# BraveGroup/DCD

Measured on NVIDIA B200. Metric: objects/sec (edge solve + GMW aggregate), higher is better.
Workload: dtype f32

## Files before the change

### dcd_b200/csrc/gmw_mlp_fused.cu

```cuda
#include <type_traits>
#include "gmw_tc_common.cuh"

#ifndef DCD_FUSED_STAT_SLEEP
#define DCD_FUSED_STAT_SLEEP 40
#endif
#ifndef DCD_FUSED_CONV_FINAL
#define DCD_FUSED_CONV_FINAL 1
#endif
#ifndef DCD_FUSED_POLL_GRACE
#define DCD_FUSED_POLL_GRACE 500
#endif
#ifndef DCD_FUSED_DONE_SLEEP
#define DCD_FUSED_DONE_SLEEP 20
#endif

namespace dcd {
#ifdef DCD_FUSED_TRACE
__device__ long long g_trace[12288];
__device__ int g_trace_n[3];
#ifndef DCD_FUSED_TRACE_CTA
#define DCD_FUSED_TRACE_CTA 0
#endif
#ifndef DCD_FUSED_TRACE_WARP
#define DCD_FUSED_TRACE_WARP 0
#endif
#define TR_DECL const bool trace_on = blockIdx.x == DCD_FUSED_TRACE_CTA && (warp == DCD_FUSED_TRACE_WARP || warp == FCONV_WARPS || warp == FCONV_WARPS + 1); int tr_k = 0;
#define TR(slot, tag)                                                       \
    do {                                                                    \
        if (trace_on && lane == 0 && tr_k < 2048) {                         \
            g_trace[(slot) * 4096 + 2 * tr_k] = (tag);                      \
            g_trace[(slot) * 4096 + 2 * tr_k + 1] = clock64();              \
            ++tr_k;                                                         \
            g_trace_n[slot] = tr_k;                                         \
        }                                                                   \
    } while (0)
#else
#define TR_DECL
#define TR(slot, tag) do { } while (0)
#endif
#if defined(DCD_FUSED_TRACE) && DCD_FUSED_TRACE + 0 >= 2
#define TRF(slot, tag) TR(slot, tag)
#else
#define TRF(slot, tag) do { } while (0)
#endif
namespace {

constexpr int FCS = 24;
constexpr int FOBJ = 3;
constexpr int FCONV_WARPS = 12;
constexpr int FCONV_THREADS = 32 * FCONV_WARPS;
constexpr int FTHREADS = FCONV_THREADS + 128;
constexpr int FSUB = 48;
constexpr int FES_MAX = 112;
constexpr uint32_t FT_W = 384;
constexpr uint32_t FB_SBO = 128;
constexpr uint32_t FB_LBO = 768;
constexpr uint32_t FB_PART = 16 * FB_LBO;

constexpr size_t SMF_X = 0;
constexpr size_t SMF_B = SMF_X + (size_t)FOBJ * FES_MAX * CH * sizeof(float);
constexpr size_t SMF_PART = SMF_B + 4 * FB_PART;
constexpr size_t SMF_BAR = SMF_PART + (FOBJ * 3 * CH + 64) * sizeof(float2);
constexpr size_t kFusedSmem = SMF_BAR + 128;
static_assert(kFusedSmem <= 232448, "shared memory budget");
static_assert(FOBJ * 6 * FES_MAX * sizeof(float) <= 4 * FB_PART, "edge features are staged in the operand buffers");
static_assert(FOBJ * FES_MAX <= FCONV_THREADS, "one converter thread per staged edge");
enum { BAR_FULL0 = 0, BAR_FULL1 = 1, BAR_DONE0 = 2, BAR_DONE1 = 3, BAR_PDONE = 4, BAR_WREADY = 5, BAR_STAT0 = 6, BAR_COUNT = 9 };
enum { NB_PART0 = 5, NB_STATW = 8 };
constexpr int FSTAT_THREADS = 96;
constexpr int NB_THREADS = FCONV_THREADS + FSTAT_THREADS;

__device__ __forceinline__ void st_flagged(float2* dst, float a, float b, uint32_t flag) {
    const uint32_t bits = (__float_as_uint(b) & 0x7fffffffu) | (flag << 31);
    const unsigned long long w = ((unsigned long long)bits << 32) | (unsigned long long)__float_as_uint(a);
    asm volatile("st.relaxed.gpu.global.b64 [%0], %1;" ::"l"(dst), "l"(w) : "memory");
}
__device__ __forceinline__ float2 ld_volatile_f2(const float2* p) {
    float2 v;
    unsigned long long w;
    asm volatile("ld.relaxed.gpu.global.b64 %0, [%1];" : "=l"(w) : "l"(p) : "memory");
    v.x = __uint_as_float((uint32_t)w);
    v.y = __uint_as_float((uint32_t)(w >> 32));
    return v;
}
__device__ __forceinline__ void ld_weights8(const uint32_t* p, uint32_t* r) {
    asm volatile("ld.global.nc.L2::evict_last.v8.b32 {%0, %1, %2, %3, %4, %5, %6, %7}, [%8];"
                 : "=r"(r[0]), "=r"(r[1]), "=r"(r[2]), "=r"(r[3]), "=r"(r[4]), "=r"(r[5]), "=r"(r[6]), "=r"(r[7])
                 : "l"(p));
}
__device__ __forceinline__ void mbar_arrive(uint64_t* bar) {
    asm volatile("mbarrier.arrive.shared::cta.b64 _, [%0];" ::"r"(smem_u32(bar)) : "memory");
}
__device__ __forceinline__ void mbar_wait_backoff(uint64_t* bar, uint32_t parity, uint32_t ns) {
    uint32_t done;
    for (;;) {
        asm volatile("{\n\t.reg .pred p;\n\tmbarrier.try_wait.parity.shared::cta.b64 p, [%1], %2;\n\tselp.u32 %0, 1, 0, p;\n\t}"
                     : "=r"(done) : "r"(smem_u32(bar)), "r"(parity) : "memory");
        if (done) break;
        if (ns) __nanosleep(ns);
    }
}
__device__ __forceinline__ void nbar_sync(int id, int count) { asm volatile("bar.sync %0, %1;" ::"r"(id), "r"(count) : "memory"); }
__device__ __forceinline__ void nbar_arrive(int id, int count) { asm volatile("bar.arrive %0, %1;" ::"r"(id), "r"(count) : "memory"); }
__device__ __forceinline__ void conv_sync() { asm volatile("bar.sync 1, %0;" ::"n"(FCONV_THREADS) : "memory"); }

__device__ __forceinline__ void tmem_ld16(uint32_t taddr, float (&v)[16]) {
    uint32_t r[16];
    asm volatile(
        "tcgen05.ld.sync.aligned.32x32b.x16.b32 "
        "{%0, %1, %2, %3, %4, %5, %6, %7, %8, %9, %10, %11, %12, %13, %14, %15}, [%16];\n\t"
        "tcgen05.wait::ld.sync.aligned;"
        : "=r"(r[0]), "=r"(r[1]), "=r"(r[2]), "=r"(r[3]), "=r"(r[4]), "=r"(r[5]), "=r"(r[6]), "=r"(r[7]), "=r"(r[8]),
          "=r"(r[9]), "=r"(r[10]), "=r"(r[11]), "=r"(r[12]), "=r"(r[13]), "=r"(r[14]), "=r"(r[15])
        : "r"(taddr)
        : "memory");
#pragma unroll
    for (int i = 0; i < 16; ++i) v[i] = __uint_as_float(r[i]);
}

__device__ __forceinline__ void tmem_ld16_issue(uint32_t taddr, uint32_t (&r)[16]) {
    asm volatile(
        "tcgen05.ld.sync.aligned.32x32b.x16.b32 "
        "{%0, %1, %2, %3, %4, %5, %6, %7, %8, %9, %10, %11, %12, %13, %14, %15}, [%16];"
        : "=r"(r[0]), "=r"(r[1]), "=r"(r[2]), "=r"(r[3]), "=r"(r[4]), "=r"(r[5]), "=r"(r[6]), "=r"(r[7]), "=r"(r[8]),
          "=r"(r[9]), "=r"(r[10]), "=r"(r[11]), "=r"(r[12]), "=r"(r[13]), "=r"(r[14]), "=r"(r[15])
        : "r"(taddr)
        : "memory");
}
__device__ __forceinline__ void tmem_ld16_wait(uint32_t (&r)[16]) {
    asm volatile("tcgen05.wait::ld.sync.aligned;"
                 : "+r"(r[0]), "+r"(r[1]), "+r"(r[2]), "+r"(r[3]), "+r"(r[4]), "+r"(r[5]), "+r"(r[6]), "+r"(r[7]), "+r"(r[8]),
                   "+r"(r[9]), "+r"(r[10]), "+r"(r[11]), "+r"(r[12]), "+r"(r[13]), "+r"(r[14]), "+r"(r[15])
                 :
                 : "memory");
}

__device__ __forceinline__ void ffma2_bc(float& d0, float& d1, float a0, float a1, float b, float c) {
    asm("{\n\t.reg .b64 a, b, c, d;\n\tmov.b64 a, {%2, %3};\n\tmov.b64 b, {%4, %4};\n\tmov.b64 c, {%5, %5};\n\t"
        "fma.rn.f32x2 d, a, b, c;\n\tmov.b64 {%0, %1}, d;\n\t}"
        : "=f"(d0), "=f"(d1) : "f"(a0), "f"(a1), "f"(b), "f"(c));
}
__device__ __forceinline__ void fsq2_acc(float& s0, float& s1, float d0, float d1) {
    asm("{\n\t.reg .b64 d, s;\n\tmov.b64 d, {%2, %3};\n\tmov.b64 s, {%0, %1};\n\t"
        "fma.rn.f32x2 s, d, d, s;\n\tmov.b64 {%0, %1}, s;\n\t}"
        : "+f"(s0), "+f"(s1) : "f"(d0), "f"(d1));
}
__device__ __forceinline__ void fadd2_acc(float& s0, float& s1, float d0, float d1) {
    asm("{\n\t.reg .b64 d, s;\n\tmov.b64 d, {%2, %3};\n\tmov.b64 s, {%0, %1};\n\t"
        "add.rn.f32x2 s, s, d;\n\tmov.b64 {%0, %1}, s;\n\t}"
        : "+f"(s0), "+f"(s1) : "f"(d0), "f"(d1));
}

__device__ __forceinline__ uint64_t smem_desc_ns(uint32_t addr, uint32_t lbo, uint32_t sbo) {
    return (uint64_t)((addr & 0x3ffffu) >> 4) | ((uint64_t)(lbo >> 4) << 16) | ((uint64_t)(sbo >> 4) << 32) | (1ull << 46);
}

__device__ __forceinline__ void split2_neg(float v0, float v1, uint32_t& hp, uint32_t& lp) {
    asm("{\n\t.reg .f16 h0, h1;\n\t.reg .f32 l0, l1;\n\t"
        "cvt.rn.f16x2.f32 %0, %3, %2;\n\t"
        "mov.b32 {h0, h1}, %0;\n\t"
        "sub.rn.f32.f16 l0, h0, %2;\n\t"
        "sub.rn.f32.f16 l1, h1, %3;\n\t"
        "cvt.rn.f16x2.f32 %1, l1, l0;\n\t}"
        : "=&r"(hp), "=r"(lp)
        : "f"(v0), "f"(v1));
}

__device__ __forceinline__ void store_unit(unsigned char* b_hi, unsigned char* b_lo, int ch, int u, const float (&v)[16]) {
    uint32_t hp[8], lp[8];
#pragma unroll
    for (int q = 0; q < 8; ++q) split2_neg(v[2 * q], v[2 * q + 1], hp[q], lp[q]);
    const uint32_t off = (uint32_t)(2 * u) * FB_SBO + (uint32_t)(ch >> 3) * FB_LBO + (uint32_t)(ch & 7) * 16u;
    *reinterpret_cast<uint4*>(b_hi + off) = make_uint4(hp[0], hp[1], hp[2], hp[3]);
    *reinterpret_cast<uint4*>(b_hi + off + FB_SBO) = make_uint4(hp[4], hp[5], hp[6], hp[7]);
    *reinterpret_cast<uint4*>(b_lo + off) = make_uint4(lp[0], lp[1], lp[2], lp[3]);
    *reinterpret_cast<uint4*>(b_lo + off + FB_SBO) = make_uint4(lp[4], lp[5], lp[6], lp[7]);
}

__device__ __forceinline__ void issue_sub_gemm(uint32_t tmem_d, uint32_t a_hi, uint32_t a_lo, uint32_t b_hi, uint32_t b_lo, int N) {
    const uint32_t idesc = (1u << 4) | (1u << 16) | ((uint32_t)(N >> 3) << 17) | ((uint32_t)(CH >> 4) << 24);
    const uint64_t d_hi = smem_desc_ns(b_hi, FB_LBO, FB_SBO), d_lo = smem_desc_ns(b_lo, FB_LBO, FB_SBO);
    uint32_t acc = 0;
#pragma unroll
    for (int term = 0; term < 3; ++term) {
        const uint32_t a = (term == 1) ? a_lo : a_hi;
        const uint64_t d = (term == 0) ? d_lo : d_hi;
        const uint32_t id = (term == 0) ? (idesc | (1u << 14)) : idesc;
#pragma unroll
        for (int ks = 0; ks < CH / 16; ++ks) {
            umma_f16_ts(tmem_d, a + ks * 8, d + (uint64_t)((ks * 2 * FB_LBO) >> 4), id, acc);
            acc = 1;
        }
    }
}

}

__global__ void __launch_bounds__(1024) fused_prep_kernel(const float* __restrict__ p4, const float* __restrict__ p6, int depth,
                                                         const float* __restrict__ fold, float2* __restrict__ scales2,
                                                         float* __restrict__ bias2, uint32_t* __restrict__ img) {
    extern __shared__ float wf_s[];
    __shared__ float red[32];
    __shared__ float scale_s;
    const int m = blockIdx.x;
    const int j = m & 1, blk = (m >> 1) % depth, net = m / (2 * depth);
    const int cin = net == 0 ? 4 : 6;
    const float* prm = net == 0 ? p4 : p6;
    const int tid = threadIdx.x;
    if (j == 0) {
        const float* F = fold + ((int64_t)net * depth + blk) * FOLD_STRIDE;
        for (int i = tid; i < CH * CH; i += 1024) wf_s[i] = F[i];
        if (tid < CH) bias2[m * CH + tid] = F[CH * CH + tid];
    } else {
        const float* W2 = prm + blob_w(cin, blk, 2);
        for (int i = tid; i < CH * CH; i += 1024) wf_s[i] = W2[i];
        if (tid < CH) bias2[m * CH + tid] = prm[blob_b(cin, blk, 2) + tid];
    }
    __syncthreads();
    float mx = 0.f;
    for (int i = tid; i < CH * CH; i += 1024) mx = fmaxf(mx, fabsf(wf_s[i]));
    mx = warp_max(mx);
    if ((tid & 31) == 0) red[tid >> 5] = mx;
    __syncthreads();
    if (tid == 0) {
        mx = 0.f;
        for (int w = 0; w < 32; ++w) mx = fmaxf(mx, red[w]);
        int e = 0;
        if (mx > 0.f) frexpf(mx, &e);
        scales2[m] = make_float2(ldexpf(1.f, 10 - e), ldexpf(1.f, e - 10));
        scale_s = ldexpf(1.f, 10 - e);
    }
    __syncthreads();
    const float scale = scale_s;
    uint32_t* out = img + (size_t)m * CH * CH;
    for (int idx = tid; idx < CH * 64; idx += 1024) {
        const int row = idx & 127, c = idx >> 7;
        const float w0 = wf_s[(2 * c) * CH + row] * scale, w1 = wf_s[(2 * c + 1) * CH + row] * scale;
        const __half h0 = __float2half_rn(w0), h1 = __float2half_rn(w1);
        const __half l0 = __float2half_rn(w0 - __half2float(h0)), l1 = __float2half_rn(w1 - __half2float(h1));
        out[(((c >> 3)) * CH + row) * 8 + (c & 7)] = (uint32_t)__half_as_ushort(h0) | ((uint32_t)__half_as_ushort(h1) << 16);
        out[((8 + (c >> 3)) * CH + row) * 8 + (c & 7)] = (uint32_t)__half_as_ushort(l0) | ((uint32_t)__half_as_ushort(l1) << 16);
    }
}

namespace {

__global__ void __launch_bounds__(FTHREADS, 1)
mlp_fused_kernel(MlpArgs a, const float2* __restrict__ scales, const float* __restrict__ bias2, const uint32_t* __restrict__ wimg,
                 float2* xg, float* __restrict__ reg_w, float4* park) {
    const WsLayout& L = a.L;
    const int tid = threadIdx.x, lane = tid & 31;
    const int warp = __shfl_sync(0xffffffffu, tid >> 5, 0);
    const int quarter = warp & 3;
    TR_DECL
    const int ch = 32 * quarter + lane;
    const uint32_t rank = blockIdx.x % FCS, group = blockIdx.x / FCS;
    const int E = L.E, EP = L.EP, depth = L.depth;
    const int upo = (E + 16 * FCS - 1) / (16 * FCS);
    const int ES = 16 * upo;
    const int ntile = upo;
    const int nphase = 2 * depth;
#if DCD_FUSED_CONV_FINAL
    const bool conv_final = upo != 4;
#endif

    extern __shared__ __align__(1024) unsigned char smem[];
    float4* Xs = reinterpret_cast<float4*>(smem + SMF_X);
    unsigned char* Bbuf = smem + SMF_B;
    float2* pbuf = reinterpret_cast<float2*>(smem + SMF_PART);
    float2* tab_s = pbuf + FOBJ * 3 * CH;
    uint64_t* bar = reinterpret_cast<uint64_t*>(smem + SMF_BAR);
    uint32_t* tmem_ptr = reinterpret_cast<uint32_t*>(smem + SMF_BAR + 8 * BAR_COUNT);

    if (tid == 0) {
        mbar_init(bar + BAR_FULL0, FCONV_WARPS);
        mbar_init(bar + BAR_FULL1, FCONV_WARPS);
        mbar_init(bar + BAR_DONE0, 1);
        mbar_init(bar + BAR_DONE1, 1);
        mbar_init(bar + BAR_PDONE, 1);
        mbar_init(bar + BAR_WREADY, 4);
        for (int o = 0; o < FOBJ; ++o) mbar_init(bar + BAR_STAT0 + o, 3);
        asm volatile("fence.mbarrier_init.release.cluster;" ::: "memory");
    }
    if (tid < 9) {
        const int o = tid / 3, k = tid % 3;
        const int vld = max(0, min(ES, E - (int)rank * ES));
        int nq = 0;
        for (int u = o * upo; u < (o + 1) * upo; ++u)
            if ((u - o * upo) % 3 == k) nq += max(0, min(16, vld - 16 * (u - o * upo)));
        tab_s[tid] = make_float2((float)nq, vld > 0 ? (float)nq / (float)vld : 0.f);
        tab_s[9 + tid] = make_float2(nq > 0 ? 1.0f / (float)nq : 0.f, 0.f);
    } else if (tid >= 32 && tid < 32 + FCS) {
        const int r = tid - 32, sb = r / 8;
        const int nr = max(0, min(ES, E - r * ES));
        const int ns = max(0, min(E, (sb + 1) * 8 * ES) - min(E, sb * 8 * ES));
        tab_s[tid] = make_float2((float)nr, ns > 0 ? (float)nr / (float)ns : 0.f);
    } else if (tid >= 56 && tid < 59) {
        const int sb = tid - 56;
        const int ns = max(0, min(E, (sb + 1) * 8 * ES) - min(E, sb * 8 * ES));
        tab_s[tid] = make_float2((float)ns, (float)ns / (float)E);
    }
    if (warp == 0) tmem_alloc(tmem_ptr, 512);
    tc_fence_before();
    __syncthreads();
    tc_fence_after();
    const uint32_t tmem_base = __shfl_sync(0xffffffffu, *tmem_ptr, 0);
    const uint32_t t_lane = tmem_base + ((uint32_t)(32 * quarter) << 16);
    const int64_t ngroups = gridDim.x / FCS;
    const bool paired = reg_w != nullptr;
    const int64_t ntrip = (L.N + FOBJ - 1) / FOBJ;
    const int64_t nlist = paired ? ntrip : 2 * ntrip;
    const int64_t nmine = nlist > (int64_t)group ? (nlist - 1 - group) / ngroups + 1 : 0;
    const int64_t nd = paired ? 2 * nmine : nmine;
    auto round_trip = [&](int64_t d) { return paired ? (int64_t)group + (d >> 1) * ngroups : ((int64_t)group + d * ngroups) >> 1; };
    auto round_net = [&](int64_t d) { return paired ? (int)(d & 1) : (int)(((int64_t)group + d * ngroups) & 1); };

    if (warp >= FCONV_WARPS) {
        uint32_t wr[64];
        auto w_load = [&](int mat, int half) {
            const uint32_t* src = wimg + (size_t)mat * CH * CH + ((size_t)(half * 8) * CH + ch) * 8;
#pragma unroll
            for (int i = 0; i < 8; ++i) ld_weights8(src + (size_t)i * CH * 8, wr + 8 * i);
        };
        auto w_store = [&](int half) {
            uint32_t t[32];
#pragma unroll
            for (int i = 0; i < 32; ++i) t[i] = wr[i];
            tmem_st32(t_lane + FT_W + 64 * half, t);
#pragma unroll
            for (int i = 0; i < 32; ++i) t[i] = wr[32 + i];
            tmem_st32(t_lane + FT_W + 64 * half + 32, t);
        };
        auto w_publish = [&]() {
            tc_wait_st();
            tc_fence_before();
            __syncwarp();
            if (lane == 0) mbar_arrive(bar + BAR_WREADY);
        };
        uint32_t g = 0;
        uint32_t fpar = 0, wpar = 0, ppar = 0;
        const int nrep = warp == FCONV_WARPS + 1 ? 2 : 1;
        const float inv_em1 = 1.0f / (float)(E - 1);
        uint32_t sxc = 0;
        auto ev_row = [&](int o) {
            const uint32_t xc = (sxc >> (2 * o)) & 3u;
            return xg + ((size_t)((group * FOBJ + o) * 2 + (xc & 1u)) * FCS) * CH;
        };
        auto ev_flag = [&](int o) { return (sxc >> (2 * o + 1)) & 1u; };
        auto ev_publish = [&](int o) {
            TR(2, 700 + o);
            nbar_sync(NB_PART0 + o, NB_THREADS);
            TR(2, 710 + o);
            float2* xrow0 = ev_row(o);
            const uint32_t flag = ev_flag(o);
            float2 tb[3];
#pragma unroll
            for (int k = 0; k < 3; ++k) tb[k] = tab_s[o * 3 + k];
            const int c0 = 32 * (warp - FCONV_WARPS - 1) + lane, c1 = 96 + lane;
            float2 q[2][3];
#pragma unroll
            for (int k = 0; k < 3; ++k) {
                q[0][k] = pbuf[(o * 3 + k) * CH + c0];
                q[1][k] = pbuf[(o * 3 + k) * CH + c1];
            }
#pragma unroll
            for (int rep = 0; rep < 2; ++rep) {
                float m = 0.f, M2 = 0.f;
#pragma unroll
                for (int k = 0; k < 3; ++k) m = fmaf(tb[k].y, q[rep][k].x, m);
#pragma unroll
                for (int k = 0; k < 3; ++k) {
                    const float dd = q[rep][k].x - m;
                    if (tb[k].x > 0.f) M2 += fmaf(tb[k].x * dd, dd, q[rep][k].y);
                }
                if (rep < nrep) st_flagged(xrow0 + rank * CH + (rep ? c1 : c0), m, M2, flag);
            }
            nbar_sync(NB_STATW, FSTAT_THREADS);
            TR(2, 720 + o);
        };
        auto ev_finish = [&](int o, bool fresh) {
            const int sb = warp - FCONV_WARPS - 1;
            const float2* xrow0 = ev_row(o) + (size_t)(8 * sb) * CH + lane;
            const uint32_t flag = ev_flag(o);
            if (fresh) __nanosleep(DCD_FUSED_POLL_GRACE);
            float2 v[4][8];
            for (;;) {
#pragma unroll
                for (int q = 0; q < 4; ++q)
#pragma unroll
                    for (int r = 0; r < 8; ++r) v[q][r] = ld_volatile_f2(xrow0 + r * CH + 32 * q);
                uint32_t bad = 0;
#pragma unroll
                for (int q = 0; q < 4; ++q)
#pragma unroll
                    for (int r = 0; r < 8; ++r) bad |= (__float_as_uint(v[q][r].y) >> 31) ^ flag;
                if (!bad) break;
                __nanosleep(64);
            }
#pragma unroll
            for (int q = 0; q < 4; ++q) {
                float mu = 0.f, M2 = 0.f;
#pragma unroll
                for (int r = 0; r < 8; ++r) mu = fmaf(tab_s[32 + 8 * sb + r].y, v[q][r].x, mu);
#pragma unroll
                for (int r = 0; r < 8; ++r) {
                    const float dd = v[q][r].x - mu;
                    M2 += fmaf(tab_s[32 + 8 * sb + r].x * dd, dd, __uint_as_float(__float_as_uint(v[q][r].y) & 0x7fffffffu));
                }
                pbuf[(o * 3 + sb) * CH + 32 * q + lane] = make_float2(mu, M2);
            }
#if DCD_FUSED_CONV_FINAL
            if (conv_final) {
                __syncwarp();
                if (lane == 0) mbar_arrive(bar + BAR_STAT0 + o);
                TR(2, 730 + o);
                sxc = (sxc & ~(3u << (2 * o))) | (((((sxc >> (2 * o)) & 3u) + 1u) & 3u) << (2 * o));
                return;
            }
#endif
            nbar_sync(NB_STATW, FSTAT_THREADS);
            for (int rep = 0; rep < nrep; ++rep) {
                const int c = rep ? 96 + lane : 32 * sb + lane;
                float2 q[3];
#pragma unroll
                for (int k = 0; k < 3; ++k) q[k] = pbuf[(o * 3 + k) * CH + c];
                float m = 0.f, M2 = 0.f;
#pragma unroll
                for (int k = 0; k < 3; ++k) m = fmaf(tab_s[56 + k].y, q[k].x, m);
#pragma unroll
                for (int k = 0; k < 3; ++k) {
                    const float dd = q[k].x - m;
                    M2 += fmaf(tab_s[56 + k].x * dd, dd, q[k].y);
                }
                const float var = M2 * inv_em1;
                const float2 st = make_float2(m, rsqrtf(var + 1e-3f));
#pragma unroll
                for (int k = 0; k < 3; ++k) pbuf[(o * 3 + k) * CH + c] = st;
            }
            __syncwarp();
            if (lane == 0) mbar_arrive(bar + BAR_STAT0 + o);
            TR(2, 730 + o);
            sxc = (sxc & ~(3u << (2 * o))) | (((((sxc >> (2 * o)) & 3u) + 1u) & 3u) << (2 * o));
        };
        if (nd > 0) {
            const int mat = round_net(0) * nphase;
            w_load(mat, 0);
            w_store(0);
            w_load(mat, 1);
            w_store(1);
            w_publish();
        }
        for (int64_t d = 0; d < nd; ++d) {
            const int mat_base = round_net(d) * nphase;
            for (int ph = 0; ph <= nphase; ++ph) {
                if (warp == FCONV_WARPS) {
                    if (ph == nphase) break;
                    TR(1, 10);
                    mbar_wait(bar + BAR_WREADY, wpar);
                    tc_fence_after();
                    TR(1, 11);
                    for (int t = 0; t < ntile; ++t, ++g) {
                        const uint32_t b = g & 1u;
                        TRF(1, 100 + t);
                        mbar_wait(bar + BAR_FULL0 + b, (fpar >> b) & 1u);
                        fpar ^= 1u << b;
                        tc_fence_after();
                        TR(1, 200 + t);
                        if (elect_one()) {
                            const uint32_t b_hi = smem_u32(Bbuf) + b * 2 * FB_PART;
                            issue_sub_gemm(tmem_base + FSUB * t, tmem_base + FT_W, tmem_base + FT_W + 64, b_hi, b_hi + FB_PART, FSUB);
                            umma_commit(bar + BAR_DONE0 + b);
                            if (t == ntile - 1) umma_commit(bar + BAR_PDONE);
                        }
                        __syncwarp();
                    }
                } else {
                    if (ph > 0) {
                        ev_publish(2);
                        ev_finish(2, true);
                    }
                    if (ph == nphase) break;
                    ev_publish(0);
                    ev_finish(0, true);
                    ev_publish(1);
                }
                wpar ^= 1u;
                const bool last_ph = ph + 1 == nphase;
                const bool more = !last_ph || d + 1 < nd;
                if (more) {
                    const int mat = last_ph ? round_net(d + 1) * nphase : mat_base + ph + 1;
#ifdef DCD_EXP_NO_WRELOAD
                    (void)mat;
                    mbar_wait(bar + BAR_PDONE, ppar);
                    tc_fence_after();
                    w_publish();
#else
                    w_load(mat, 0);
                    TR(warp == FCONV_WARPS ? 1 : 2, 20);
                    mbar_wait(bar + BAR_PDONE, ppar);
                    tc_fence_after();
                    TR(warp == FCONV_WARPS ? 1 : 2, 21);
                    w_store(0);
                    w_load(mat, 1);
                    w_store(1);
                    w_publish();
#endif
                    TR(warp == FCONV_WARPS ? 1 : 2, 22);
                } else {
                    mbar_wait(bar + BAR_PDONE, ppar);
                }
                ppar ^= 1u;
                if (warp != FCONV_WARPS) ev_finish(1, false);
            }
        }
    } else {
        const int wg = warp >> 2;
        const int e_base = (int)rank * ES;
        const int valid = max(0, min(ES, E - e_base));
        uint32_t g = 0;
        uint32_t par = 0, pend = 0;
        auto wait_buf = [&](uint32_t b) {
            if ((pend >> b) & 1u) {
                mbar_wait_backoff(bar + BAR_DONE0 + b, (par >> b) & 1u, DCD_FUSED_DONE_SLEEP);
                par ^= 1u << b;
                pend &= ~(1u << b);
                tc_fence_after();
            }
        };
        auto obj_of = [&](int u) { return (u >= upo ? 1 : 0) + (u >= 2 * upo ? 1 : 0); };
        uint32_t spar = 0;
#if DCD_FUSED_CONV_FINAL
        const float inv_em1_c = 1.0f / (float)(E - 1);
#endif
        uint32_t firstmask = 0, lastmask = 0;
        for (int t = 0; t < ntile; ++t) {
            const int u = 3 * t + wg;
            if (t == 0 || obj_of(u) != obj_of(u - 3)) firstmask |= 1u << t;
            if (t == ntile - 1 || obj_of(u + 3) != obj_of(u)) lastmask |= 1u << t;
        }
        auto stream_of = [&](int o) { return (wg + 3 * o * upo - o * upo) % 3; };

        for (int64_t d = 0; d < nd; ++d) {
            const int64_t trip = round_trip(d);
            const int net = round_net(d);
            const int64_t obj0 = FOBJ * trip;
            const int cin = net == 0 ? 4 : 6;
            const float* __restrict__ prm = a.params[net];
            const int mat_base = net * nphase;

            TR(0, 900);
            wait_buf(0);
            wait_buf(1);
            conv_sync();
            float* f_s = reinterpret_cast<float*>(Bbuf);
            if (tid < FOBJ * ES) {
                const int o = obj_of(tid >> 4);
                const int el = tid - o * ES;
                const int e = e_base + el;
                const int64_t obj = min(obj0 + o, L.N - 1);
                int i, j;
                decode_edge(e < E ? e : E - 1, L.n, i, j);
                float f[6];
                if (net == 0) {
                    const float2 pi = __ldg(reinterpret_cast<const float2*>(a.kpts2d + (obj * L.n + i) * 2));
                    const float2 pj = __ldg(reinterpret_cast<const float2*>(a.kpts2d + (obj * L.n + j) * 2));
                    f[0] = pi.x; f[1] = pi.y; f[2] = pj.x; f[3] = pj.y; f[4] = 0.f; f[5] = 0.f;
                } else {
                    const float* pi = a.kpts3d + (obj * L.n + i) * 3;
                    const float* pj = a.kpts3d + (obj * L.n + j) * 3;
                    f[0] = __ldg(pi); f[1] = __ldg(pi + 1); f[2] = __ldg(pi + 2);
                    f[3] = __ldg(pj); f[4] = __ldg(pj + 1); f[5] = __ldg(pj + 2);
                }
#pragma unroll
                for (int r = 0; r < 6; ++r) f_s[(o * 6 + r) * ES + el] = f[r];
            }
            conv_sync();
            {
                float wq[6];
#pragma unroll
                for (int q = 0; q < 6; ++q) wq[q] = (q < cin) ? __ldg(prm + blob_in_w() + q * CH + ch) : 0.f;
                const float b = __ldg(prm + blob_in_b(cin) + ch);
                for (int u = wg; u < FOBJ * upo; u += 3) {
                    const int o = obj_of(u);
                    const int lc = 16 * (u - o * upo);
                    const float* fo = f_s + o * 6 * ES + lc;
#pragma unroll
                    for (int q4 = 0; q4 < 4; ++q4) {
                        float x[4];
#pragma unroll
                        for (int i = 0; i < 4; ++i) {
                            const int e = 4 * q4 + i;
                            float acc = b;
#pragma unroll
                            for (int r = 0; r < 6; ++r) acc = fmaf(wq[r], fo[r * ES + e], acc);
                            x[i] = (lc + e < valid) ? acc : 0.f;
                        }
                        Xs[(4 * u + q4) * CH + ch] = make_float4(x[0], x[1], x[2], x[3]);
                    }
                }
            }
            conv_sync();
            TR(0, 901);

            float un_out = 0.f, b_out = 0.f, un_prev = 0.f, b_prev = 0.f;
            float un_next = __ldg(scales + mat_base).y, b_next = __ldg(bias2 + mat_base * CH + ch);
            int npend = 0, t_e = 0, o_e = 0, ob_e = 0, p_e = 0;
            float K = 0.f, s1 = 0.f, s2 = 0.f, bK = 0.f;
            bool have_K = false;
            uint32_t cv[16], sv[16];

            auto stats_math = [&](const uint32_t (&raw)[16], int nv, float un, float bb) {
                if (!have_K) {
                    K = fmaf(__uint_as_float(raw[0]), un, bb);
                    bK = bb - K;
                    have_K = true;
                }
                if (nv >= 16) {
                    float t1[4] = {0.f, 0.f, 0.f, 0.f}, t2[4] = {0.f, 0.f, 0.f, 0.f};
#pragma unroll
                    for (int i = 0; i < 16; i += 4) {
                        float d0, d1, d2, d3;
                        ffma2_bc(d0, d1, __uint_as_float(raw[i]), __uint_as_float(raw[i + 1]), un, bK);
                        ffma2_bc(d2, d3, __uint_as_float(raw[i + 2]), __uint_as_float(raw[i + 3]), un, bK);
                        fadd2_acc(t1[0], t1[1], d0, d1);
                        fadd2_acc(t1[2], t1[3], d2, d3);
                        fsq2_acc(t2[0], t2[1], d0, d1);
                        fsq2_acc(t2[2], t2[3], d2, d3);
                    }
                    s1 += (t1[0] + t1[1]) + (t1[2] + t1[3]);
                    s2 += (t2[0] + t2[1]) + (t2[2] + t2[3]);
                } else {
#pragma unroll
                    for (int i = 0; i < 16; ++i)
                        if (i < nv) {
                            const float dd = fmaf(__uint_as_float(raw[i]), un, bK);
                            s1 += dd;
                            s2 = fmaf(dd, dd, s2);
                        }
                }
            };
            auto post = [&](int o) {
                const int k = stream_of(o);
                const float ic = tab_s[9 + o * 3 + k].x;
                const float m = K + s1 * ic;
                const float M2 = fmaxf(fmaf(-s1 * ic, s1, s2), 0.f);
                pbuf[(o * 3 + k) * CH + ch] = make_float2(m, M2);
                nbar_arrive(NB_PART0 + o, NB_THREADS);
                TR(0, 603);
                K = 0.f; s1 = 0.f; s2 = 0.f; bK = 0.f;
                have_K = false;
            };
            auto collect = [&](int o) {
                TR(0, 606);
                mbar_wait_backoff(bar + BAR_STAT0 + o, (spar >> o) & 1u, DCD_FUSED_STAT_SLEEP);
                spar ^= 1u << o;
                TR(0, 608);
#if DCD_FUSED_CONV_FINAL
                if (conv_final) {
                    float2 q[3];
#pragma unroll
                    for (int k = 0; k < 3; ++k) q[k] = pbuf[(o * 3 + k) * CH + ch];
                    float m = 0.f, M2 = 0.f;
#pragma unroll
                    for (int k = 0; k < 3; ++k) m = fmaf(tab_s[56 + k].y, q[k].x, m);
#pragma unroll
                    for (int k = 0; k < 3; ++k) {
                        const float dd = q[k].x - m;
                        M2 += fmaf(tab_s[56 + k].x * dd, dd, q[k].y);
                    }
                    return make_float2(m, rsqrtf(M2 * inv_em1_c + 1e-3f));
                }
#endif
                return pbuf[(o * 3 + stream_of(o)) * CH + ch];
            };
            auto process_due = [&](bool loaded, int ph) {
                const int cb = FSUB * t_e + 16 * wg;
                const int nv = valid - (cb - ob_e);
                if (nv > 0) {
                    if (!loaded) {
                        tmem_ld16_issue(t_lane + cb, sv);
                        tmem_ld16_wait(sv);
                    }
                    const bool cur = p_e == (ph & 1);
                    stats_math(sv, nv, cur ? un_out : un_prev, cur ? b_out : b_prev);
                }
                if ((lastmask >> t_e) & 1u) post(o_e);
                if (++t_e == ntile) {
                    t_e = 0; o_e = 0; ob_e = 0; p_e ^= 1;
                } else if ((firstmask >> t_e) & 1u) {
                    ++o_e; ob_e += ES;
                }
            };

            float a_in = 0.f, c_in = 0.f;
            for (int ph = 0; ph < nphase; ++ph) {
                const int kind = (ph & 1) ? 2 : 0;
                un_prev = un_out;
                b_prev = b_out;
                un_out = un_next;
                b_out = b_next;
                if (ph + 1 < nphase) {
                    un_next = __ldg(scales + mat_base + ph + 1).y;
                    b_next = __ldg(bias2 + (mat_base + ph + 1) * CH + ch);
                }
                const bool reads_d = ph > 0;
                int o = 0, ob = 0;
                for (int t = 0; t < ntile; ++t, ++g) {
                    const int cb = FSUB * t + 16 * wg;
                    if ((firstmask >> t) & 1u) {
                        if (t > 0) { ++o; ob += ES; }
                        if (reads_d) {
                            const float2 st = collect(o);
                            a_in = un_prev * st.y;
                            c_in = (b_prev - st.x) * st.y;
                        }
                    }
                    const int lc = cb - ob;
                    const uint32_t b = g & 1u;
                    TR(0, 1000 * kind + 100 + t);
                    wait_buf(b);
                    TRF(0, 1000 * kind + 200 + t);
                    unsigned char* b_hi = Bbuf + (size_t)b * 2 * FB_PART;
                    const bool due = npend == 2;
                    const int cb_e = FSUB * t_e + 16 * wg;
                    const bool st_load = due && valid > cb_e - ob_e;
                    float v[16];
                    float4* Xp = Xs + (cb >> 2) * CH + ch;
                    float4 x4[4];
                    if (kind == 0) {
#pragma unroll
                        for (int q4 = 0; q4 < 4; ++q4) x4[q4] = Xp[q4 * CH];
                    }
                    if (reads_d) tmem_ld16_wait(cv);
                    TRF(0, 1000 * kind + 300 + t);
                    if (st_load) tmem_ld16_issue(t_lane + cb_e, sv);
                    if (kind == 0) {
                        if (reads_d) {
#pragma unroll
                            for (int i = 0; i < 16; i += 2) {
                                ffma2_bc(v[i], v[i + 1], __uint_as_float(cv[i]), __uint_as_float(cv[i + 1]), a_in, c_in);
                                v[i] = fmaxf(v[i], 0.f);
                                v[i + 1] = fmaxf(v[i + 1], 0.f);
                            }
#pragma unroll
                            for (int q4 = 0; q4 < 4; ++q4) {
                                fadd2_acc(v[4 * q4], v[4 * q4 + 1], x4[q4].x, x4[q4].y);
                                fadd2_acc(v[4 * q4 + 2], v[4 * q4 + 3], x4[q4].z, x4[q4].w);
                            }
                            if (lc + 16 > valid) {
#pragma unroll
                                for (int i = 0; i < 16; ++i)
                                    if (lc + i >= valid) v[i] = 0.f;
                            }
#pragma unroll
                            for (int q4 = 0; q4 < 4; ++q4)
                                Xp[q4 * CH] = make_float4(v[4 * q4], v[4 * q4 + 1], v[4 * q4 + 2], v[4 * q4 + 3]);
                        } else {
#pragma unroll
                            for (int q4 = 0; q4 < 4; ++q4) {
                                v[4 * q4] = x4[q4].x; v[4 * q4 + 1] = x4[q4].y; v[4 * q4 + 2] = x4[q4].z; v[4 * q4 + 3] = x4[q4].w;
                            }
                        }
                    } else {
#pragma unroll
                        for (int i = 0; i < 16; i += 2)
                            ffma2_bc(v[i], v[i + 1], __uint_as_float(cv[i]), __uint_as_float(cv[i + 1]), a_in, c_in);
                    }
                    store_unit(b_hi, b_hi + FB_PART, ch, wg, v);
                    TRF(0, 1000 * kind + 400 + t);
                    fence_async_smem();
                    tc_fence_before();
                    __syncwarp();
                    if (lane == 0) mbar_arrive(bar + BAR_FULL0 + b);
                    pend |= 1u << b;
                    TRF(0, 1000 * kind + 500 + t);
                    if (st_load) tmem_ld16_wait(sv);
                    if (t + 1 < ntile) {
                        if (reads_d) tmem_ld16_issue(t_lane + cb + FSUB, cv);
                    } else if (ph + 1 < nphase) {
                        tmem_ld16_issue(t_lane + 16 * wg, cv);
                    }
                    if (due) process_due(true, ph); else ++npend;
                }
            }
            TR(0, 600);

            wait_buf(0);
            wait_buf(1);
            un_prev = un_out;
            b_prev = b_out;
            while (npend > 0) {
                process_due(false, nphase);
                --npend;
            }
            TR(0, 601);
            int o_cur = -1;
            float a_fin = 0.f, c_fin = 0.f;
            int itn = 0;
            for (int u = wg; u < FOBJ * upo; u += 3, ++itn) {
                const int o = obj_of(u);
                const int lc = 16 * (u - o * upo);
                if (o != o_cur) {
                    const float2 st = collect(o);
                    a_fin = un_out * st.y;
                    c_fin = (b_out - st.x) * st.y;
                    o_cur = o;
                }
                const bool emit = obj0 + o < L.N;
                const int64_t obj = min(obj0 + o, L.N - 1);
                float v[16];
                {
                    const float4* Xp = Xs + (4 * u) * CH + ch;
                    float4 x4[4];
#pragma unroll
                    for (int q4 = 0; q4 < 4; ++q4) x4[q4] = Xp[q4 * CH];
                    tmem_ld16(t_lane + 16 * u, v);
#pragma unroll
                    for (int i = 0; i < 16; ++i) v[i] = fmaxf(fmaf(v[i], a_fin, c_fin), 0.f);
#pragma unroll
                    for (int q4 = 0; q4 < 4; ++q4) {
                        v[4 * q4] += x4[q4].x; v[4 * q4 + 1] += x4[q4].y; v[4 * q4 + 2] += x4[q4].z; v[4 * q4 + 3] += x4[q4].w;
                    }
                    if (lc + 16 > valid) {
#pragma unroll
                        for (int i = 0; i < 16; ++i)
                            if (lc + i >= valid) v[i] = 0.f;
                    }
                }
                if (!paired) {
                    float* G = act_ptr(a.ws, L, net, 0, SLOT_X) + obj * (int64_t)CH * EP + (int64_t)ch * EP;
#pragma unroll
                    for (int q4 = 0; q4 < 4; ++q4)
                        if (emit && e_base + lc + 4 * q4 < EP)
                            __stcs(reinterpret_cast<float4*>(G + e_base + lc + 4 * q4), make_float4(v[4 * q4], v[4 * q4 + 1], v[4 * q4 + 2], v[4 * q4 + 3]));
                } else if (net == 0) {
                    float4* Pk = park + ((size_t)blockIdx.x * (4 * FOBJ * upo) + 4 * u) * CH + ch;
#pragma unroll
                    for (int q4 = 0; q4 < 4; ++q4) Pk[q4 * CH] = make_float4(v[4 * q4], v[4 * q4 + 1], v[4 * q4 + 2], v[4 * q4 + 3]);
                } else {
                    const float4* Pk = park + ((size_t)blockIdx.x * (4 * FOBJ * upo) + 4 * u) * CH + ch;
                    float* red = reinterpret_cast<float*>(Bbuf) + wg * (2 * 4 * 48);
                    float* W = reg_w + obj * (int64_t)E + e_base + lc;
                    float aa[16], cc[16], ac[16];
#pragma unroll
                    for (int q4 = 0; q4 < 4; ++q4) {
                        const float4 p = Pk[q4 * CH];
                        const float av[4] = {p.x, p.y, p.z, p.w};
#pragma unroll
                        for (int i = 0; i < 4; ++i) {
                            const float c = v[4 * q4 + i];
                            aa[4 * q4 + i] = __fmul_rn(av[i], av[i]);
                            cc[4 * q4 + i] = __fmul_rn(c, c);
                            ac[4 * q4 + i] = __fmul_rn(av[i], c);
                        }
                    }
#pragma unroll
                    for (int h = 8; h >= 1; h >>= 1) {
                        const bool up = (lane & (2 * h)) != 0;
#pragma unroll
                        for (int k = 0; k < h; ++k) {
                            const float sa = up ? aa[k] : aa[k + h], sc = up ? cc[k] : cc[k + h], sx = up ? ac[k] : ac[k + h];
                            const float ka = up ? aa[k + h] : aa[k], kc = up ? cc[k + h] : cc[k], kx = up ? ac[k + h] : ac[k];
                            aa[k] = __fadd_rn(ka, __shfl_xor_sync(0xffffffffu, sa, 2 * h));
                            cc[k] = __fadd_rn(kc, __shfl_xor_sync(0xffffffffu, sc, 2 * h));
                            ac[k] = __fadd_rn(kx, __shfl_xor_sync(0xffffffffu, sx, 2 * h));
                        }
                    }
                    aa[0] = __fadd_rn(aa[0], __shfl_xor_sync(0xffffffffu, aa[0], 1));
                    cc[0] = __fadd_rn(cc[0], __shfl_xor_sync(0xffffffffu, cc[0], 1));
                    ac[0] = __fadd_rn(ac[0], __shfl_xor_sync(0xffffffffu, ac[0], 1));
                    float* rb = red + (itn & 1) * (4 * 48);
                    if ((lane & 1) == 0) {
                        float* op = rb + quarter * 48 + (lane >> 1) * 3;
                        op[0] = aa[0]; op[1] = cc[0]; op[2] = ac[0];
                    }
                    asm volatile("bar.sync %0, 128;" ::"r"(2 + wg) : "memory");
                    if (quarter == 0 && lane < 16) {
                        if (lc + lane < valid && emit) {
                            const float* op = rb + lane * 3;
                            const float saa = __fadd_rn(__fadd_rn(op[0], op[48]), __fadd_rn(op[96], op[144]));
                            const float scc = __fadd_rn(__fadd_rn(op[1], op[49]), __fadd_rn(op[97], op[145]));
                            const float sac = __fadd_rn(__fadd_rn(op[2], op[50]), __fadd_rn(op[98], op[146]));
                            const float n4 = fmaxf(sqrtf(saa), 1e-12f), n6 = fmaxf(sqrtf(scc), 1e-12f);
                            const float a2 = __fdiv_rn(saa, __fmul_rn(n4, n4)), c2 = __fdiv_rn(scc, __fmul_rn(n6, n6));
                            const float acn = __fdiv_rn(sac, __fmul_rn(n4, n6));
                            const float s2w = __fadd_rn(__fadd_rn(c2, -2.f * acn), a2);
                            W[lane] = __fdiv_rn(1.f, sqrtf(fmaxf(s2w, 1e-30f)));
                        }
                    }
                }
            }
            TR(0, 610);
            tc_fence_before();
        }
    }
    tc_fence_before();
    __syncthreads();
    if (warp == 0) tmem_dealloc(tmem_base, 512);
}

}

#ifdef DCD_FUSED_TRACE
}
extern "C" __attribute__((visibility("default"))) int dcd_debug_fused_trace(long long* dst, int* n) {
    cudaDeviceSynchronize();
    cudaMemcpyFromSymbol(dst, dcd::g_trace, sizeof(long long) * 12288);
    cudaMemcpyFromSymbol(n, dcd::g_trace_n, sizeof(int) * 3);
    return 0;
}
namespace dcd {
#endif

bool gmw_fused_supported(int n) {
    const int E = n * (n - 1) / 2;
    const int upo = (E + 16 * FCS - 1) / (16 * FCS);
    return upo >= 3 && 16 * upo <= FES_MAX;
}

constexpr int FMAX_GROUPS = 10;
constexpr size_t kExchangeBytes = (size_t)FMAX_GROUPS * FOBJ * 2 * FCS * CH * sizeof(float2);

static size_t fused_scales_bytes(int depth) { return (((size_t)4 * depth * sizeof(float2)) + 255) / 256 * 256; }
static size_t fused_bias_bytes(int depth) { return (size_t)4 * depth * CH * sizeof(float); }
static size_t fused_image_only_bytes(int depth) { return (size_t)4 * depth * CH * CH * sizeof(uint32_t); }
size_t gmw_fused_image_bytes(int depth) {
    return fused_scales_bytes(depth) + fused_bias_bytes(depth) + fused_image_only_bytes(depth) + kExchangeBytes;
}

int launch_gmw_fused_fwd(const MlpArgs& a, const float* params4, const float* params6, void* tail, float* reg_w, bool* emitted,
                         cudaStream_t st) {
    const int depth = a.L.depth;
    unsigned char* base = reinterpret_cast<unsigned char*>(tail);
    float2* scales2 = reinterpret_cast<float2*>(base);
    float* bias2 = reinterpret_cast<float*>(base + fused_scales_bytes(depth));
    uint32_t* wimg = reinterpret_cast<uint32_t*>(base + fused_scales_bytes(depth) + fused_bias_bytes(depth));
    float2* xg = reinterpret_cast<float2*>(base + fused_scales_bytes(depth) + fused_bias_bytes(depth) + fused_image_only_bytes(depth));
    int dev = 0;
    if (cudaGetDevice(&dev) != cudaSuccess) return DCD_E_DEVICE;
    cudaFuncSetAttribute(mlp_fused_kernel, cudaFuncAttributeMaxDynamicSharedMemorySize, (int)kFusedSmem);
    cudaFuncSetAttribute(fused_prep_kernel, cudaFuncAttributeMaxDynamicSharedMemorySize, (int)(CH * CH * sizeof(float)));
    int coop = 0, per_sm = 0;
    cudaDeviceGetAttribute(&coop, cudaDevAttrCooperativeLaunch, dev);
    cudaOccupancyMaxActiveBlocksPerMultiprocessor(&per_sm, mlp_fused_kernel, FTHREADS, kFusedSmem);
    if (!coop || per_sm < 1) return DCD_E_UNSUPPORTED;
    int max_groups = device_sm_count() * per_sm / FCS;
    if (max_groups > FMAX_GROUPS) max_groups = FMAX_GROUPS;
    if (max_groups < 1) return DCD_E_UNSUPPORTED;
    fused_prep_kernel<<<4 * depth, 1024, CH * CH * sizeof(float), st>>>(params4, params6, depth, a.fold, scales2, bias2, wimg);
    cudaMemsetAsync(xg, 0x80, kExchangeBytes, st);
    const int64_t es = 16 * ((a.L.E + 16 * FCS - 1) / (16 * FCS));
    const bool paired = reg_w != nullptr && a.L.N >= FOBJ * (int64_t)max_groups &&
                        a.L.N * (int64_t)a.L.EP >= (int64_t)max_groups * FOBJ * FCS * es;
    const int64_t npairs = (a.L.N + FOBJ - 1) / FOBJ;
    const int64_t nitems = paired ? npairs : npairs * 2;
    const int ngroups = (int)(nitems < max_groups ? nitems : max_groups);
    MlpArgs args = a;
    const float2* scales_arg = scales2;
    const float* bias_arg = bias2;
    const uint32_t* wimg_arg = wimg;
    float* regw_arg = paired ? reg_w : nullptr;
    float4* park_arg = reinterpret_cast<float4*>(act_ptr(a.ws, a.L, 0, 0, SLOT_Y1));
    void* kargs[] = {&args, &scales_arg, &bias_arg, &wimg_arg, &xg, &regw_arg, &park_arg};
    if (cudaLaunchCooperativeKernel(reinterpret_cast<void*>(mlp_fused_kernel), dim3(FCS * ngroups), dim3(FTHREADS), kargs, kFusedSmem,
                                    st) != cudaSuccess) {
        cudaGetLastError();
        return DCD_E_LAUNCH;
    }
    *emitted = paired;
    return DCD_OK;
}

}
```

Baseline: 51970.

## Stream next-layer weights into a TMEM ring to overlap reload with MMAs

Replaces the all-at-once weight reload, which waited for every MMA of a phase to finish, with a 22-slot TMEM ring of 8-column weight chunks. A constexpr rotation table decides which slots hold hi, lo and the next layer's first chunks. Stores into those slots are gated by new barriers (a lo-done commit and two wready barriers), so the next layer's weights are written while the current layer's MMAs still run. This hides the reload stall between phases, at the cost of more barrier traffic, more complex parity tracking and a higher risk of ordering bugs.

```diff
diff --git a/dcd_b200/csrc/gmw_mlp_fused.cu b/dcd_b200/csrc/gmw_mlp_fused.cu
--- a/dcd_b200/csrc/gmw_mlp_fused.cu
+++ b/dcd_b200/csrc/gmw_mlp_fused.cu
@@ -12,6 +12,9 @@
 #endif
 #ifndef DCD_FUSED_DONE_SLEEP
 #define DCD_FUSED_DONE_SLEEP 20
+#endif
+#ifndef DCD_FUSED_FULL_SLEEP
+#define DCD_FUSED_FULL_SLEEP 0
 #endif
 
 namespace dcd {
@@ -52,7 +55,9 @@
 constexpr int FTHREADS = FCONV_THREADS + 128;
 constexpr int FSUB = 48;
 constexpr int FES_MAX = 112;
-constexpr uint32_t FT_W = 384;
+constexpr uint32_t FT_W = FOBJ * FES_MAX;
+constexpr int FW_SLOTS = (512 - FT_W) / 8;
+static_assert(FW_SLOTS == 22, "the ring holds one layer's 16 weight chunks and the next layer's first 6");
 constexpr uint32_t FB_SBO = 128;
 constexpr uint32_t FB_LBO = 768;
 constexpr uint32_t FB_PART = 16 * FB_LBO;
@@ -65,7 +70,8 @@
 static_assert(kFusedSmem <= 232448, "shared memory budget");
 static_assert(FOBJ * 6 * FES_MAX * sizeof(float) <= 4 * FB_PART, "edge features are staged in the operand buffers");
 static_assert(FOBJ * FES_MAX <= FCONV_THREADS, "one converter thread per staged edge");
-enum { BAR_FULL0 = 0, BAR_FULL1 = 1, BAR_DONE0 = 2, BAR_DONE1 = 3, BAR_PDONE = 4, BAR_WREADY = 5, BAR_STAT0 = 6, BAR_COUNT = 9 };
+enum { BAR_FULL0 = 0, BAR_FULL1 = 1, BAR_DONE0 = 2, BAR_DONE1 = 3, BAR_PDONE = 4, BAR_LODONE = 5, BAR_WREADY0 = 6, BAR_WREADY1 = 7,
+       BAR_STAT0 = 8, BAR_COUNT = 11 };
 enum { NB_PART0 = 5, NB_STATW = 8 };
 constexpr int FSTAT_THREADS = 96;
 constexpr int NB_THREADS = FCONV_THREADS + FSTAT_THREADS;
@@ -177,20 +183,57 @@
     *reinterpret_cast<uint4*>(b_lo + off + FB_SBO) = make_uint4(lp[4], lp[5], lp[6], lp[7]);
 }
 
-__device__ __forceinline__ void issue_sub_gemm(uint32_t tmem_d, uint32_t a_hi, uint32_t a_lo, uint32_t b_hi, uint32_t b_lo, int N) {
+template <int N> using IC = std::integral_constant<int, N>;
+
+__device__ __forceinline__ void tmem_st8(uint32_t taddr, const uint32_t* r) {
+    asm volatile("tcgen05.st.sync.aligned.32x32b.x8.b32 [%0], {%1, %2, %3, %4, %5, %6, %7, %8};" ::"r"(taddr), "r"(r[0]), "r"(r[1]),
+                 "r"(r[2]), "r"(r[3]), "r"(r[4]), "r"(r[5]), "r"(r[6]), "r"(r[7])
+                 : "memory");
+}
+
+constexpr int FW_PERIOD = 11;
+struct WRingTable { uint32_t w[FW_PERIOD + 1][6]; };
+constexpr WRingTable make_wring_table() {
+    WRingTable t{};
+    int h[8] = {0, 1, 2, 3, 4, 5, 6, 7}, l[8] = {8, 9, 10, 11, 12, 13, 14, 15}, f[8] = {16, 17, 18, 19, 20, 21, 0, 0};
+    for (int k = 0; k <= FW_PERIOD; ++k) {
+        for (int i = 0; i < 8; ++i) {
+            t.w[k][i >> 2] |= (uint32_t)h[i] << (8 * (i & 3));
+            t.w[k][2 + (i >> 2)] |= (uint32_t)l[i] << (8 * (i & 3));
+            if (i < 6) t.w[k][4 + (i >> 2)] |= (uint32_t)f[i] << (8 * (i & 3));
+        }
+        const int nh[8] = {f[0], f[1], f[2], f[3], f[4], f[5], l[0], l[1]}, nl[8] = {l[2], l[3], l[4], l[5], l[6], l[7], h[0], h[1]};
+        for (int i = 0; i < 6; ++i) f[i] = h[2 + i];
+        for (int i = 0; i < 8; ++i) { h[i] = nh[i]; l[i] = nl[i]; }
+    }
+    return t;
+}
+constexpr WRingTable kWRingHost = make_wring_table();
+static_assert(kWRingHost.w[FW_PERIOD][0] == kWRingHost.w[0][0] && kWRingHost.w[FW_PERIOD][1] == kWRingHost.w[0][1] &&
+              kWRingHost.w[FW_PERIOD][2] == kWRingHost.w[0][2] && kWRingHost.w[FW_PERIOD][3] == kWRingHost.w[0][3] &&
+              kWRingHost.w[FW_PERIOD][4] == kWRingHost.w[0][4] && kWRingHost.w[FW_PERIOD][5] == kWRingHost.w[0][5],
+              "the ring's period");
+__constant__ WRingTable kWRing = kWRingHost;
+struct WRing {
+    uint32_t k = 0;
+    __device__ uint32_t slot(int word, int i) const { return (kWRing.w[k][word] >> (8 * i)) & 0xffu; }
+    __device__ uint32_t hi(int ks) const { return slot(ks >> 2, ks & 3); }
+    __device__ uint32_t lo(int ks) const { return slot(2 + (ks >> 2), ks & 3); }
+    __device__ uint32_t fr(int i) const { return slot(4 + (i >> 2), i & 3); }
+    __device__ void advance() { k = k + 1 == FW_PERIOD ? 0 : k + 1; }
+};
+
+template <int I0, int I1>
+__device__ __forceinline__ void issue_mmas(uint32_t tmem_d, uint32_t t_w, const WRing& w, uint32_t b_hi, uint32_t b_lo, int N) {
     const uint32_t idesc = (1u << 4) | (1u << 16) | ((uint32_t)(N >> 3) << 17) | ((uint32_t)(CH >> 4) << 24);
     const uint64_t d_hi = smem_desc_ns(b_hi, FB_LBO, FB_SBO), d_lo = smem_desc_ns(b_lo, FB_LBO, FB_SBO);
-    uint32_t acc = 0;
-#pragma unroll
-    for (int term = 0; term < 3; ++term) {
-        const uint32_t a = (term == 1) ? a_lo : a_hi;
+#pragma unroll
+    for (int i = I0; i < I1; ++i) {
+        const int term = i >> 3, ks = i & 7;
+        const uint32_t a = t_w + 8 * (term == 1 ? w.lo(ks) : w.hi(ks));
         const uint64_t d = (term == 0) ? d_lo : d_hi;
         const uint32_t id = (term == 0) ? (idesc | (1u << 14)) : idesc;
-#pragma unroll
-        for (int ks = 0; ks < CH / 16; ++ks) {
-            umma_f16_ts(tmem_d, a + ks * 8, d + (uint64_t)((ks * 2 * FB_LBO) >> 4), id, acc);
-            acc = 1;
-        }
+        umma_f16_ts(tmem_d, a, d + (uint64_t)((ks * 2 * FB_LBO) >> 4), id, i > 0 ? 1u : 0u);
     }
 }
 
@@ -278,7 +321,9 @@
         mbar_init(bar + BAR_DONE0, 1);
         mbar_init(bar + BAR_DONE1, 1);
         mbar_init(bar + BAR_PDONE, 1);
-        mbar_init(bar + BAR_WREADY, 4);
+        mbar_init(bar + BAR_LODONE, 1);
+        mbar_init(bar + BAR_WREADY0, 4);
+        mbar_init(bar + BAR_WREADY1, 4);
         for (int o = 0; o < FOBJ; ++o) mbar_init(bar + BAR_STAT0 + o, 3);
         asm volatile("fence.mbarrier_init.release.cluster;" ::: "memory");
     }
@@ -317,28 +362,19 @@
 
     if (warp >= FCONV_WARPS) {
         uint32_t wr[64];
-        auto w_load = [&](int mat, int half) {
-            const uint32_t* src = wimg + (size_t)mat * CH * CH + ((size_t)(half * 8) * CH + ch) * 8;
-#pragma unroll
-            for (int i = 0; i < 8; ++i) ld_weights8(src + (size_t)i * CH * 8, wr + 8 * i);
+        auto w_ld = [&](int mat, int c0, auto nc, auto i0) {
+            const uint32_t* src = wimg + (size_t)mat * CH * CH + ((size_t)c0 * CH + ch) * 8;
+#pragma unroll
+            for (int i = 0; i < decltype(nc)::value; ++i) ld_weights8(src + (size_t)i * CH * 8, wr + 8 * (i + decltype(i0)::value));
         };
-        auto w_store = [&](int half) {
-            uint32_t t[32];
-#pragma unroll
-            for (int i = 0; i < 32; ++i) t[i] = wr[i];
-            tmem_st32(t_lane + FT_W + 64 * half, t);
-#pragma unroll
-            for (int i = 0; i < 32; ++i) t[i] = wr[32 + i];
-            tmem_st32(t_lane + FT_W + 64 * half + 32, t);
-        };
-        auto w_publish = [&]() {
+        auto w_st = [&](int i, uint32_t s) { tmem_st8(t_lane + FT_W + 8 * s, wr + 8 * i); };
+        auto w_publish = [&](int b) {
             tc_wait_st();
             tc_fence_before();
             __syncwarp();
-            if (lane == 0) mbar_arrive(bar + BAR_WREADY);
+            if (lane == 0) mbar_arrive(bar + b);
         };
-        uint32_t g = 0;
-        uint32_t fpar = 0, wpar = 0, ppar = 0;
+        WRing ring;
         const int nrep = warp == FCONV_WARPS + 1 ? 2 : 1;
         const float inv_em1 = 1.0f / (float)(E - 1);
         uint32_t sxc = 0;
@@ -444,73 +480,144 @@
         };
         if (nd > 0) {
             const int mat = round_net(0) * nphase;
-            w_load(mat, 0);
-            w_store(0);
-            w_load(mat, 1);
-            w_store(1);
-            w_publish();
+            w_ld(mat, 0, IC<8>(), IC<0>());
+#pragma unroll
+            for (int i = 0; i < 8; ++i) w_st(i, ring.hi(i));
+            w_ld(mat, 8, IC<8>(), IC<0>());
+#pragma unroll
+            for (int i = 0; i < 8; ++i) w_st(i, ring.lo(i));
+            w_publish(BAR_WREADY0);
+            if (lane == 0) mbar_arrive(bar + BAR_WREADY1);
         }
-        for (int64_t d = 0; d < nd; ++d) {
-            const int mat_base = round_net(d) * nphase;
-            for (int ph = 0; ph <= nphase; ++ph) {
-                if (warp == FCONV_WARPS) {
-                    if (ph == nphase) break;
-                    TR(1, 10);
-                    mbar_wait(bar + BAR_WREADY, wpar);
-                    tc_fence_after();
-                    TR(1, 11);
+        auto store_a = [&]() {
+#pragma unroll
+            for (int i = 0; i < 6; ++i) w_st(i, ring.fr(i));
+        };
+        auto store_b = [&]() {
+#pragma unroll
+            for (int i = 0; i < 8; ++i) w_st(i, ring.lo(i));
+            ring.advance();
+            w_publish(BAR_WREADY0);
+        };
+        auto store_c = [&]() {
+            w_st(0, ring.lo(6));
+            w_st(1, ring.lo(7));
+            w_publish(BAR_WREADY1);
+        };
+        auto next_mat = [&](int64_t d, int ph) { return ph + 1 < nphase ? round_net(d) * nphase + ph + 1 : round_net(d + 1) * nphase; };
+        if (warp == FCONV_WARPS) {
+            uint32_t g = 0;
+            uint32_t fpar = 0, ppar = 0, lpar = 0, w0par = 0, w1par = 0;
+            bool lo_due = false;
+            for (int64_t d = 0; d < nd; ++d) {
+                for (int ph = 0; ph < nphase; ++ph) {
+                    const bool more = ph + 1 < nphase || d + 1 < nd;
+                    const int nmat = more ? next_mat(d, ph) : 0;
                     for (int t = 0; t < ntile; ++t, ++g) {
                         const uint32_t b = g & 1u;
+                        const uint32_t b_hi = smem_u32(Bbuf) + b * 2 * FB_PART;
+                        const uint32_t tmem_d = tmem_base + FSUB * t, t_w = tmem_base + FT_W;
                         TRF(1, 100 + t);
-                        mbar_wait(bar + BAR_FULL0 + b, (fpar >> b) & 1u);
+                        mbar_wait_backoff(bar + BAR_FULL0 + b, (fpar >> b) & 1u, DCD_FUSED_FULL_SLEEP);
                         fpar ^= 1u << b;
+                        TR(1, 200 + t);
+                        if (t == 0) {
+                            TR(1, 10);
+                            mbar_wait(bar + BAR_WREADY0, w0par);
+                            w0par ^= 1u;
+                            TR(1, 11);
+                        }
                         tc_fence_after();
-                        TR(1, 200 + t);
+                        if (elect_one()) issue_mmas<0, 14>(tmem_d, t_w, ring, b_hi, b_hi + FB_PART, FSUB);
+                        __syncwarp();
+                        if (t == 0) {
+                            if (lo_due) {
+                                TR(1, 20);
+                                mbar_wait(bar + BAR_PDONE, ppar);
+                                ppar ^= 1u;
+                                tc_fence_after();
+                                TR(1, 21);
+                                store_c();
+                                lo_due = false;
+                                TR(1, 22);
+                            }
+                            TR(1, 12);
+                            mbar_wait(bar + BAR_WREADY1, w1par);
+                            w1par ^= 1u;
+                            tc_fence_after();
+                            TR(1, 13);
+                        }
                         if (elect_one()) {
-                            const uint32_t b_hi = smem_u32(Bbuf) + b * 2 * FB_PART;
-                            issue_sub_gemm(tmem_base + FSUB * t, tmem_base + FT_W, tmem_base + FT_W + 64, b_hi, b_hi + FB_PART, FSUB);
+                            issue_mmas<14, 16>(tmem_d, t_w, ring, b_hi, b_hi + FB_PART, FSUB);
+                            if (t == ntile - 1) umma_commit(bar + BAR_LODONE);
+                            issue_mmas<16, 24>(tmem_d, t_w, ring, b_hi, b_hi + FB_PART, FSUB);
                             umma_commit(bar + BAR_DONE0 + b);
                             if (t == ntile - 1) umma_commit(bar + BAR_PDONE);
                         }
                         __syncwarp();
-                    }
-                } else {
+                        if (more && t == 0) w_ld(nmat, 0, IC<6>(), IC<0>());
+                        if (more && t == 1) {
+                            store_a();
+                            TR(1, 25);
+                            w_ld(nmat, 6, IC<8>(), IC<0>());
+                        }
+                    }
+                    if (more) {
+                        TR(1, 23);
+                        mbar_wait(bar + BAR_LODONE, lpar);
+                        lpar ^= 1u;
+                        tc_fence_after();
+                        TR(1, 24);
+                        store_b();
+                        w_ld(nmat, 14, IC<2>(), IC<0>());
+                        lo_due = true;
+                    } else {
+                        mbar_wait(bar + BAR_PDONE, ppar);
+                    }
+                }
+            }
+        } else {
+            uint32_t ppar = 0, lpar = 0;
+            for (int64_t d = 0; d < nd; ++d) {
+                for (int ph = 0; ph <= nphase; ++ph) {
                     if (ph > 0) {
                         ev_publish(2);
                         ev_finish(2, true);
                     }
                     if (ph == nphase) break;
+                    const bool more = ph + 1 < nphase || d + 1 < nd;
+                    const int nmat = more ? next_mat(d, ph) : 0;
+                    if (more) w_ld(nmat, 0, IC<4>(), IC<0>());
                     ev_publish(0);
+                    if (more) {
+                        w_ld(nmat, 4, IC<2>(), IC<4>());
+                        store_a();
+                        TR(2, 25);
+                    }
                     ev_finish(0, true);
+                    if (more) w_ld(nmat, 6, IC<4>(), IC<0>());
                     ev_publish(1);
-                }
-                wpar ^= 1u;
-                const bool last_ph = ph + 1 == nphase;
-                const bool more = !last_ph || d + 1 < nd;
-                if (more) {
-                    const int mat = last_ph ? round_net(d + 1) * nphase : mat_base + ph + 1;
-#ifdef DCD_EXP_NO_WRELOAD
-                    (void)mat;
+                    if (more) {
+                        w_ld(nmat, 10, IC<4>(), IC<4>());
+                        TR(2, 23);
+                        mbar_wait(bar + BAR_LODONE, lpar);
+                        lpar ^= 1u;
+                        tc_fence_after();
+                        TR(2, 24);
+                        store_b();
+                        w_ld(nmat, 14, IC<2>(), IC<0>());
+                    }
+                    TR(2, 20);
                     mbar_wait(bar + BAR_PDONE, ppar);
+                    ppar ^= 1u;
                     tc_fence_after();
-                    w_publish();
-#else
-                    w_load(mat, 0);
-                    TR(warp == FCONV_WARPS ? 1 : 2, 20);
-                    mbar_wait(bar + BAR_PDONE, ppar);
-                    tc_fence_after();
-                    TR(warp == FCONV_WARPS ? 1 : 2, 21);
-                    w_store(0);
-                    w_load(mat, 1);
-                    w_store(1);
-                    w_publish();
-#endif
-                    TR(warp == FCONV_WARPS ? 1 : 2, 22);
-                } else {
-                    mbar_wait(bar + BAR_PDONE, ppar);
-                }
-                ppar ^= 1u;
-                if (warp != FCONV_WARPS) ev_finish(1, false);
+                    TR(2, 21);
+                    if (more) {
+                        store_c();
+                        TR(2, 22);
+                    }
+                    ev_finish(1, false);
+                }
             }
         }
     } else {
```

Result: faster. 52710 (median of 6 runs) (+1.4%).
